# eth-ait/MultiPly

Measured on NVIDIA H100. Metric: rays/sec, higher is better.
Workload: dtype f32 (fp16 hi/lo split tensor-core operands, fp32 accumulate)

## Files before the change

### multiply_b200/csrc/mlp_tc.cu

```cuda
#include "common.cuh"
#include <vector>
#include <mutex>
#include <type_traits>
#include <stdlib.h>

namespace mp {

enum {
  K_SP_PLAIN = 0,
  K_SP_SAVE = 1,
  K_SP_SEED = 2,
  K_FEAT = 3,
  K_BWD = 4,
  K_FINAL_GRAD = 5,
  K_RELU = 6
};
enum {
  F_INJECT_EMB = 1,
  F_SDF_DOT = 2,
  F_SKIP_GRAD = 4,
  F_EXTRA_IN = 8,
  F_RGB_OUT = 16
};
constexpr int kMaxSteps = 24;
constexpr int kSlotBytes = 32768;
constexpr int kRing = 3;
constexpr int kBlobSlots = 170;

struct TcStep {
  int nk;
  int kind;
  int flags;
  int sig;
  const float* bias;
  int slot_off;
  int sc;
  int terms;
};

struct TcProgram {
  int nsteps;
  TcStep step[kMaxSteps];
  const uint4* blob;
  const float* inv_scale;
  int d_in, multires, E, inj_col, n_extra;
  const float* w8row;
  const float* b8;
  const float* Wrgb;
  const float* brgb;
};

struct TcIO : MlpCall {
  float rz;
  char* scratch;
  size_t scratch_per_cta;
};

constexpr int kConsumers = 2;
constexpr int kThreads = 128 * (1 + kConsumers);

constexpr size_t kSigBytes = (size_t)8 * kConsumers * 32 * 128 * 16;
constexpr size_t kFeatBytes = (size_t)kConsumers * 32 * 128 * 16;
constexpr size_t kGeBytes = (size_t)96 * 128 * 4;
constexpr size_t kEmbBytes = (size_t)96 * 128 * 4;
constexpr size_t kScratchPerCta = kSigBytes + kFeatBytes + kGeBytes + kEmbBytes;

constexpr int kABytes = 2 * 4 * 128 * 128;
constexpr int kSmemBytes = kABytes + kRing * kSlotBytes + 256 + 1024;
static_assert(kSmemBytes <= 232448, "shared memory budget of one CTA (227 KB)");

__device__ __forceinline__ uint32_t smem_u32(const void* p) { return (uint32_t)__cvta_generic_to_shared(p); }

__device__ __forceinline__ void mbar_init(uint64_t* bar, uint32_t count) {
  asm volatile("mbarrier.init.shared::cta.b64 [%0], %1;" ::"r"(smem_u32(bar)), "r"(count));
}
__device__ __forceinline__ void mbar_arrive(uint64_t* bar) {
  asm volatile("mbarrier.arrive.shared::cta.b64 _, [%0];" ::"r"(smem_u32(bar)) : "memory");
}
__device__ __forceinline__ void mbar_expect_tx(uint64_t* bar, uint32_t bytes) {
  asm volatile("mbarrier.arrive.expect_tx.shared::cta.b64 _, [%0], %1;" ::"r"(smem_u32(bar)), "r"(bytes) : "memory");
}
__device__ __forceinline__ void mbar_wait(uint64_t* bar, uint32_t parity) {
  asm volatile(
      "{\n"
      ".reg .pred p;\n"
      "WAIT_LOOP:\n"
      "mbarrier.try_wait.parity.shared::cta.b64 p, [%0], %1;\n"
      "@p bra WAIT_DONE;\n"
      "bra WAIT_LOOP;\n"
      "WAIT_DONE:\n"
      "}\n" ::"r"(smem_u32(bar)),
      "r"(parity)
      : "memory");
}
__device__ __forceinline__ void bulk_g2s(void* dst, const void* src, uint32_t bytes, uint64_t* bar) {
  asm volatile("cp.async.bulk.shared::cluster.global.mbarrier::complete_tx::bytes [%0], [%1], %2, [%3];" ::"r"(
                   smem_u32(dst)),
               "l"(src), "r"(bytes), "r"(smem_u32(bar))
               : "memory");
}
__device__ __forceinline__ void prefetch_l2(const void* p, uint32_t bytes) {
  asm volatile("cp.async.bulk.prefetch.L2.global [%0], %1;" ::"l"(p), "r"(bytes) : "memory");
}
__device__ __forceinline__ void fence_async_smem() { asm volatile("fence.proxy.async.shared::cta;" ::: "memory"); }

__device__ __forceinline__ void wg_sync(int id) { asm volatile("bar.sync %0, 128;" ::"r"(id) : "memory"); }

__device__ __forceinline__ void wgmma_fence() { asm volatile("wgmma.fence.sync.aligned;" ::: "memory"); }
__device__ __forceinline__ void wgmma_commit() { asm volatile("wgmma.commit_group.sync.aligned;" ::: "memory"); }
template <int N>
__device__ __forceinline__ void wgmma_wait() {
  asm volatile("wgmma.wait_group.sync.aligned %0;" ::"n"(N) : "memory");
}
__device__ __forceinline__ void acc_fence(float* d) {
#pragma unroll
  for (int i = 0; i < 128; ++i) asm volatile("" : "+f"(d[i])::"memory");
}

#define MP_D4(i) "+f"(d[i]), "+f"(d[i + 1]), "+f"(d[i + 2]), "+f"(d[i + 3])
#define MP_D16(i) MP_D4(i), MP_D4(i + 4), MP_D4(i + 8), MP_D4(i + 12)
__device__ __forceinline__ void wgmma_f16(float* d, uint64_t a_desc, uint64_t b_desc, uint32_t accumulate) {
  asm volatile(
      "{\n"
      ".reg .pred p;\n"
      "setp.ne.b32 p, %130, 0;\n"
      "wgmma.mma_async.sync.aligned.m64n256k16.f32.f16.f16 "
      "{%0, %1, %2, %3, %4, %5, %6, %7, %8, %9, %10, %11, %12, %13, %14, %15, "
      "%16, %17, %18, %19, %20, %21, %22, %23, %24, %25, %26, %27, %28, %29, %30, %31, "
      "%32, %33, %34, %35, %36, %37, %38, %39, %40, %41, %42, %43, %44, %45, %46, %47, "
      "%48, %49, %50, %51, %52, %53, %54, %55, %56, %57, %58, %59, %60, %61, %62, %63, "
      "%64, %65, %66, %67, %68, %69, %70, %71, %72, %73, %74, %75, %76, %77, %78, %79, "
      "%80, %81, %82, %83, %84, %85, %86, %87, %88, %89, %90, %91, %92, %93, %94, %95, "
      "%96, %97, %98, %99, %100, %101, %102, %103, %104, %105, %106, %107, %108, %109, %110, %111, "
      "%112, %113, %114, %115, %116, %117, %118, %119, %120, %121, %122, %123, %124, %125, %126, %127}, "
      "%128, %129, p, 1, 1, 0, 0;\n"
      "}\n"
      : MP_D16(0), MP_D16(16), MP_D16(32), MP_D16(48), MP_D16(64), MP_D16(80), MP_D16(96), MP_D16(112)
      : "l"(a_desc), "l"(b_desc), "r"(accumulate));
}
#undef MP_D16
#undef MP_D4

__device__ __forceinline__ uint64_t make_desc(uint32_t saddr) {
  return (uint64_t)((saddr >> 4) & 0x3FFF) | (1ull << 16) | ((uint64_t)(1024 >> 4) << 32) | (1ull << 62);
}

__device__ __forceinline__ uint32_t a_off(int row, int kb, int ch) {
  return (uint32_t)(kb * 16384 + row * 128 + ((ch ^ (row & 7)) << 4));
}

__device__ __forceinline__ void split2(float a, float b, uint32_t& hi, uint32_t& lo) {
  __half2 h = __floats2half2_rn(a, b);
  float2 f = __half22float2(h);
  __half2 l = __floats2half2_rn(a - f.x, b - f.y);
  hi = *(uint32_t*)&h;
  lo = *(uint32_t*)&l;
}
__device__ __forceinline__ void split8(const float* v, uint4& hi, uint4& lo) {
  split2(v[0], v[1], hi.x, lo.x);
  split2(v[2], v[3], hi.y, lo.y);
  split2(v[4], v[5], hi.z, lo.z);
  split2(v[6], v[7], hi.w, lo.w);
}

__device__ __forceinline__ void sts128(uint32_t A32, uint32_t off, const uint4& v) {
  asm volatile("st.shared.v4.b32 [%0], {%1, %2, %3, %4};" ::"r"(A32 + off), "r"(v.x), "r"(v.y), "r"(v.z), "r"(v.w));
}
__device__ __forceinline__ void store_a8(uint32_t A32, int row, int col, const float* v) {
  uint4 hi, lo;
  split8(v, hi, lo);
  uint32_t o = a_off(row, col >> 6, (col >> 3) & 7);
  sts128(A32, o, hi);
  sts128(A32, 65536 + o, lo);
}
__device__ __forceinline__ void stsm4(uint32_t addr, uint32_t a, uint32_t b, uint32_t c, uint32_t e) {
  asm volatile("stmatrix.sync.aligned.m8n8.x4.shared.b16 [%0], {%1, %2, %3, %4};" ::"r"(addr), "r"(a), "r"(b), "r"(c),
               "r"(e));
}
__device__ __forceinline__ void store_pairs(uint32_t lane_base, uint32_t lane_x, int jp, const uint4& hi, const uint4& lo) {
  const uint32_t addr = lane_base + (uint32_t)(jp >> 2) * 16384u + ((((uint32_t)(2 * jp) & 7u) ^ lane_x) << 4);
  stsm4(addr, hi.x, hi.y, hi.z, hi.w);
  stsm4(addr + 65536u, lo.x, lo.y, lo.z, lo.w);
}
__device__ __forceinline__ void store_acc16(uint32_t lane_base, uint32_t lane_x, int jp, const float* v) {
  uint4 hi, lo;
  split8(v, hi, lo);
  store_pairs(lane_base, lane_x, jp, hi, lo);
}

__device__ __forceinline__ float quad_sum(float v) {
  v += __shfl_xor_sync(0xffffffffu, v, 1);
  v += __shfl_xor_sync(0xffffffffu, v, 2);
  return v;
}

__device__ __forceinline__ float4 ld_stream(const float4* p) {
  float4 v;
  asm volatile("ld.global.cg.v4.f32 {%0,%1,%2,%3}, [%4];" : "=f"(v.x), "=f"(v.y), "=f"(v.z), "=f"(v.w) : "l"(p));
  return v;
}
__device__ __forceinline__ uint4 ld_stream(const uint4* p) {
  uint4 v;
  asm volatile("ld.global.cg.v4.u32 {%0,%1,%2,%3}, [%4];" : "=r"(v.x), "=r"(v.y), "=r"(v.z), "=r"(v.w) : "l"(p));
  return v;
}
__device__ __forceinline__ void st_stream(float4* p, const float4& v) {
  asm volatile("st.global.cg.v4.f32 [%0], {%1,%2,%3,%4};" ::"l"(p), "f"(v.x), "f"(v.y), "f"(v.z), "f"(v.w) : "memory");
}
__device__ __forceinline__ void st_stream(uint4* p, const uint4& v) {
  asm volatile("st.global.cg.v4.u32 [%0], {%1,%2,%3,%4};" ::"l"(p), "r"(v.x), "r"(v.y), "r"(v.z), "r"(v.w) : "memory");
}

__device__ __forceinline__ void discard_line(const void* p, float dep) {
  asm volatile("discard.global.L2 [%0], 128;" ::"l"(p), "f"(dep) : "memory");
}
__device__ __forceinline__ void discard_line(const void* p, uint32_t dep) {
  asm volatile("discard.global.L2 [%0], 128;" ::"l"(p), "r"(dep) : "memory");
}

__device__ __forceinline__ float ex2_approx(float x) {
  float y;
  asm("ex2.approx.ftz.f32 %0, %1;" : "=f"(y) : "f"(x));
  return y;
}
__device__ __forceinline__ float lg2_approx(float x) {
  float y;
  asm("lg2.approx.ftz.f32 %0, %1;" : "=f"(y) : "f"(x));
  return y;
}
__device__ __forceinline__ float rcp_approx(float x) {
  float y;
  asm("rcp.approx.ftz.f32 %0, %1;" : "=f"(y) : "f"(x));
  return y;
}
__device__ __forceinline__ float softplus_fast(float z) {
  float t = z * 144.26950408889634f;
  float u = ex2_approx(t);
  float y = lg2_approx(1.f + u) * 0.0069314718055994531f;
  return t > 28.853900817779268f ? z : y;
}
__device__ __forceinline__ void softplus_fast_grad(float z, float& y, float& d) {
  float t = z * 144.26950408889634f;
  float u = ex2_approx(t);
  float w = 1.f + u;
  float r = rcp_approx(w);
  float ys = lg2_approx(w) * 0.0069314718055994531f;
  bool big = t > 28.853900817779268f;
  y = big ? z : ys;
  d = big ? 1.f : u * r;
}

__device__ __forceinline__ void final_grad(const TcProgram& P, const TcIO& io, const float* acc, float isc, int q,
                                           const float* ge, const float* emb, const int (&rowt)[2],
                                           const bool (&valid)[2], const int (&pt)[2], const int (&slot)[2],
                                           float (&nrm)[2][3]) {
  const int d = P.d_in;
  float gax[2][4] = {{0.f, 0.f, 0.f, 0.f}, {0.f, 0.f, 0.f, 0.f}};
  const int nterm = 1 + 2 * P.multires;
#pragma unroll
  for (int j = 0; j < 8; ++j) {
    if (j < 2 * d) {
      const int a = j >> 1;
#pragma unroll
      for (int e = 0; e < 4; ++e) {
        const int jj = (8 * j + 2 * q + (e & 1)) & 15;
        if (jj < nterm) {
          const int h = e >> 1;
          const int fq = (jj - 1) >> 1;
          const bool is_cos = ((jj - 1) & 1) != 0;
          const int k = (jj == 0) ? a : d + 2 * fq * d + (is_cos ? d : 0) + a;
          const float pg = ge[(size_t)k * 128 + rowt[h]];
          const float tot = fmaf(acc[4 * j + e], isc, pg);
          float w = 1.f;
          if (jj > 0) {
            const float pe = emb[(size_t)(is_cos ? k - d : k + d) * 128 + rowt[h]];
            w = (float)(1 << fq) * (is_cos ? -pe : pe);
          }
          gax[h][a] = fmaf(w, tot, gax[h][a]);
        }
      }
    }
  }
#pragma unroll
  for (int h = 0; h < 2; ++h) {
#pragma unroll
    for (int a = 0; a < 4; ++a) gax[h][a] = quad_sum(gax[h][a]);
    const float gx0 = gax[h][0], gx1 = d > 1 ? gax[h][1] : 0.f, gx2 = d > 2 ? gax[h][2] : 0.f;
    if (q == 0 && io.grad && valid[h]) {
      io.grad[3 * (size_t)pt[h]] = gx0;
      io.grad[3 * (size_t)pt[h] + 1] = gx1;
      io.grad[3 * (size_t)pt[h] + 2] = gx2;
    }
    float n0 = 0.f, n1 = 0.f, n2 = 0.f;
    if (io.jinv && valid[h]) {
      const float4* J4 = (const float4*)(io.jinv + 12 * (size_t)pt[h]);
      const float4 ja = __ldg(J4), jb = __ldg(J4 + 1), jc = __ldg(J4 + 2);
      float v0 = gx0 * ja.x + gx1 * ja.w + gx2 * jb.z;
      float v1 = gx0 * ja.y + gx1 * jb.x + gx2 * jb.w;
      float v2 = gx0 * ja.z + gx1 * jb.y + gx2 * jc.x;
      float nr = fmaxf(sqrtf(v0 * v0 + v1 * v1 + v2 * v2), 1e-12f);
      const float inr = 1.f / nr;
      v0 *= inr; v1 *= inr; v2 *= inr;
      float n2r = fmaxf(sqrtf(v0 * v0 + v1 * v1 + v2 * v2), 1e-6f);
      const float in2 = 1.f / n2r;
      n0 = v0 * in2; n1 = v1 * in2; n2 = v2 * in2;
      if (q == 0 && io.nrm) {
        io.nrm[3 * (size_t)slot[h]] = n0;
        io.nrm[3 * (size_t)slot[h] + 1] = n1;
        io.nrm[3 * (size_t)slot[h] + 2] = n2;
      }
    }
    nrm[h][0] = n0;
    nrm[h][1] = n1;
    nrm[h][2] = n2;
  }
}

__global__ void __launch_bounds__(kThreads, 1) tc_chain_kernel(const __grid_constant__ TcProgram P,
                                                               const __grid_constant__ TcIO io) {
  extern __shared__ uint8_t smem_raw[];
  const int warp = threadIdx.x >> 5, lane = threadIdx.x & 31;
  char* base = (char*)(((uintptr_t)smem_raw + 1023) & ~(uintptr_t)1023);
  char* A = base;
  const uint32_t A32 = smem_u32(A);
  char* ring = base + kABytes;
  uint64_t* bars = (uint64_t*)(ring + kRing * kSlotBytes);
  uint64_t* full = bars;
  uint64_t* empty = bars + kRing;

  const int count = io.count ? min(io.cap, *io.count) : io.cap;
  const int ntiles = (count + 127) >> 7;

  if (threadIdx.x == 0) {
    for (int i = 0; i < kRing; ++i) {
      mbar_init(&full[i], 1);
      mbar_init(&empty[i], 4 * kConsumers);
    }
    asm volatile("fence.mbarrier_init.release.cluster;" ::: "memory");
  }
  __syncthreads();

  if (warp < 4) {
    asm volatile("setmaxnreg.dec.sync.aligned.u32 40;\n" ::: "memory");
    if (warp == 0 && lane == 0) {
      uint32_t it = 0;
      for (int tile = blockIdx.x; tile < ntiles; tile += gridDim.x) {
        for (int s = 0; s < P.nsteps; ++s) {
          const char* src = (const char*)P.blob + (size_t)P.step[s].slot_off * kSlotBytes;
          const int nslot = 2 * P.step[s].nk;
          const int jstep = P.step[s].terms == 1 ? 2 : 1;
          for (int j = 0; j < nslot; j += jstep, ++it) {
            int r = it % kRing;
            uint32_t ph = (it / kRing) & 1;
            mbar_wait(&empty[r], ph ^ 1);
            mbar_expect_tx(&full[r], kSlotBytes);
            bulk_g2s(ring + (size_t)r * kSlotBytes, src + (size_t)j * kSlotBytes, kSlotBytes, &full[r]);
          }
        }
      }
    }
    return;
  }
  asm volatile("setmaxnreg.inc.sync.aligned.u32 232;\n" ::: "memory");
  const int g = (warp >> 2) - 1;
  const int t = threadIdx.x & 127;
  const int wq = warp & 3, q = lane & 3;
  const int bar_id = 1 + g;
  int rowt[2];
  rowt[0] = 64 * g + 16 * wq + (lane >> 2);
  rowt[1] = rowt[0] + 8;
  const int mi = lane >> 3, rr = lane & 7;
  const uint32_t lane_base = A32 + (uint32_t)(64 * g + 16 * wq + 8 * (mi & 1) + rr) * 128u;
  const uint32_t lane_x = (uint32_t)((mi >> 1) ^ rr);
  const uint32_t a_hi = A32 + (uint32_t)g * 8192u, a_lo = a_hi + 65536u;

  char* scr = io.scratch + (size_t)blockIdx.x * io.scratch_per_cta;
  float4* sig = (float4*)scr;
  uint4* fsc = (uint4*)(scr + kSigBytes) + (size_t)g * 32 * 128;
  float* ge = (float*)(scr + kSigBytes + kFeatBytes);
  float* emb = (float*)(scr + kSigBytes + kFeatBytes + kGeBytes);
  const int d = P.d_in, E = P.E;

  float acc[128];
#pragma unroll
  for (int i = 0; i < 128; ++i) acc[i] = 0.f;
  uint32_t it = 0;

  for (int tile = blockIdx.x; tile < ntiles; tile += gridDim.x) {
    int pt[2], slot[2];
    bool valid[2];
    float x[2][4];
#pragma unroll
    for (int h = 0; h < 2; ++h) {
      pt[h] = tile * 128 + rowt[h];
      valid[h] = pt[h] < count;
      for (int a = 0; a < 4; ++a) x[h][a] = 0.f;
      if (valid[h])
        for (int a = 0; a < d; ++a) x[h][a] = io.x[(size_t)pt[h] * d + a];
      slot[h] = valid[h] ? (io.slot ? io.slot[pt[h]] : pt[h]) : 0;
    }
    {
      const int npair = d * P.multires;
      for (int pi = q; pi < npair; pi += 4) {
        const int f = pi / d, a = pi - f * d;
#pragma unroll
        for (int h = 0; h < 2; ++h) {
          float sn, cs;
          sincosf(__fmul_rn(x[h][a], (float)(1 << f)), &sn, &cs);
          emb[(size_t)(d + 2 * f * d + a) * 128 + rowt[h]] = sn;
          emb[(size_t)(d + (2 * f + 1) * d + a) * 128 + rowt[h]] = cs;
        }
      }
      if (q == 0)
        for (int a = 0; a < d; ++a)
#pragma unroll
          for (int h = 0; h < 2; ++h) emb[(size_t)a * 128 + rowt[h]] = x[h][a];
      if (io.dirs) {
        float dv[2][3];
#pragma unroll
        for (int h = 0; h < 2; ++h)
          for (int a = 0; a < 3; ++a) dv[h][a] = valid[h] ? io.dirs[(size_t)pt[h] * 3 + a] : 0.f;
        const int nvp = (P.n_extra - 3) / 2;
        for (int pi = q; pi < nvp; pi += 4) {
          const int f = pi / 3, a = pi - f * 3;
#pragma unroll
          for (int h = 0; h < 2; ++h) {
            float sn, cs;
            sincosf(__fmul_rn(dv[h][a], (float)(1 << f)), &sn, &cs);
            ge[(size_t)(3 + 6 * f + a) * 128 + rowt[h]] = sn;
            ge[(size_t)(3 + 6 * f + 3 + a) * 128 + rowt[h]] = cs;
          }
        }
        if (q == 0)
          for (int a = 0; a < 3; ++a)
#pragma unroll
            for (int h = 0; h < 2; ++h) ge[(size_t)a * 128 + rowt[h]] = dv[h][a];
      }
      __threadfence_block();
      wg_sync(bar_id);
      const int njp = P.step[0].nk * 4;
      for (int jp = 0; jp < njp; ++jp) {
        float v[8];
#pragma unroll
        for (int i = 0; i < 8; ++i) {
          const int c = 16 * jp + 8 * (i >> 2) + 2 * q + (i & 1);
          v[i] = (c < E) ? emb[(size_t)c * 128 + rowt[(i >> 1) & 1]] : 0.f;
        }
        store_acc16(lane_base, lane_x, jp, v);
      }
    }
    float nrm[2][3] = {{0.f, 0.f, 0.f}, {0.f, 0.f, 0.f}};
    for (int s = 0; s < P.nsteps; ++s) {
      const TcStep st = P.step[s];
      const float isc = P.inv_scale[st.sc] * fmaf(io.rz, (float)(4 * st.nk * (st.terms == 1 ? 1 : 3)), 1.f);
      const bool one_term = st.terms == 1;
      if (t == 0) {
        char* ws = io.scratch + (size_t)blockIdx.x * io.scratch_per_cta;
        if (st.kind == K_BWD && st.sig >= 0)
          prefetch_l2(ws + (((size_t)st.sig * kConsumers + g) * 32 * 128) * 16, 32 * 128 * 16);
        if (st.kind == K_FINAL_GRAD) prefetch_l2(ws + kSigBytes + (size_t)g * 32 * 128 * 16, 32 * 128 * 16);
      }

      fence_async_smem();
      wg_sync(bar_id);
      wgmma_fence();
      bool held = false;
      uint32_t held_slot = 0;
      auto release = [&](uint32_t slot_it) {
        if (lane == 0) mbar_arrive(&empty[slot_it % kRing]);
      };
      auto slot_issued = [&](uint32_t slot_it) {
        wgmma_commit();
        if (held) {
          wgmma_wait<1>();
          release(held_slot);
        }
        held = true;
        held_slot = slot_it;
      };
      for (int kc = 0; kc < st.nk; ++kc) {
        if (kc == 4) {
          wgmma_wait<0>();
          acc_fence(acc);
          if (held) release(held_slot);
          held = false;
#pragma unroll
          for (int h = 0; h < 2; ++h) {
#pragma unroll
            for (int c8 = 0; c8 < 16; c8 += 8) {
              const int e0 = 16 * q + c8;
              float xv[8];
#pragma unroll
              for (int j = 0; j < 8; ++j) xv[j] = 0.f;
              if (io.dirs) {
#pragma unroll
                for (int j = 0; j < 8; ++j)
                  if (e0 + j < P.n_extra) xv[j] = ge[(size_t)(e0 + j) * 128 + rowt[h]];
              } else if (e0 == 0) {
                xv[0] = x[h][0]; xv[1] = x[h][1]; xv[2] = x[h][2];
                xv[3] = nrm[h][0]; xv[4] = nrm[h][1]; xv[5] = nrm[h][2];
              }
              store_a8(A32, rowt[h], e0, xv);
            }
          }
          fence_async_smem();
          wg_sync(bar_id);
          wgmma_fence();
        }
        const uint32_t ka = (uint32_t)(kc & 3) * 16384u;
        int r = it % kRing;
        mbar_wait(&full[r], (it / kRing) & 1);
        uint32_t wb = smem_u32(ring + (size_t)r * kSlotBytes);
#pragma unroll
        for (int ks = 0; ks < 4; ++ks) {
          const uint64_t bd = make_desc(wb + ks * 32);
          wgmma_f16(acc, make_desc(a_hi + ka + ks * 32), bd, (kc | ks) != 0);
          if (!one_term) wgmma_f16(acc, make_desc(a_lo + ka + ks * 32), bd, 1);
        }
        slot_issued(it++);
        if (!one_term) {
          r = it % kRing;
          mbar_wait(&full[r], (it / kRing) & 1);
          wb = smem_u32(ring + (size_t)r * kSlotBytes);
#pragma unroll
          for (int ks = 0; ks < 4; ++ks) wgmma_f16(acc, make_desc(a_hi + ka + ks * 32), make_desc(wb + ks * 32), 1);
          slot_issued(it++);
        }
      }
      wgmma_wait<0>();
      acc_fence(acc);
      if (held) release(held_slot);

      auto reload_features = [&]() {
#pragma unroll
        for (int jp = 0; jp < 16; ++jp) {
          const uint4 fh = ld_stream(&fsc[(size_t)jp * 128 + t]);
          const uint4 fl = ld_stream(&fsc[(size_t)(16 + jp) * 128 + t]);
          store_pairs(lane_base, lane_x, jp, fh, fl);
          if ((lane & 7) == 0) {
            discard_line(&fsc[(size_t)jp * 128 + t], fh.x);
            discard_line(&fsc[(size_t)(16 + jp) * 128 + t], fl.x);
          }
        }
      };
      if (st.kind == K_FINAL_GRAD) {
        final_grad(P, io, acc, isc, q, ge, emb, rowt, valid, pt, slot, nrm);
        if (s + 1 < P.nsteps) reload_features();
        continue;
      }

      auto run_epi = [&](auto kind) {
        constexpr int KIND = decltype(kind)::value;
        float dot[2][3] = {{0.f, 0.f, 0.f}, {0.f, 0.f, 0.f}};
#pragma unroll
        for (int jp = 0; jp < 16; ++jp) {
          float* v = acc + 8 * jp;
          float yv[8];
#pragma unroll
          for (int jj = 0; jj < 2; ++jj) {
            const int j = 2 * jp + jj;
            const int c = 8 * j + 2 * q;
            float* u = v + 4 * jj;
            float b[2] = {0.f, 0.f};
            if constexpr (KIND != K_BWD) {
              const float2 b2 = __ldg((const float2*)(st.bias + c));
              b[0] = b2.x;
              b[1] = b2.y;
            }
            if constexpr (KIND == K_SP_SEED) {
              const float2 w2 = __ldg((const float2*)(P.w8row + c));
              const float w[2] = {w2.x, w2.y};
#pragma unroll
              for (int e = 0; e < 4; ++e) {
                float y, dd;
                softplus_fast_grad(fmaf(u[e], isc, b[e & 1]), y, dd);
                dot[e >> 1][0] = fmaf(y, w[e & 1], dot[e >> 1][0]);
                yv[4 * jj + e] = y;
                u[e] = dd * w[e & 1];
              }
            } else if constexpr (KIND == K_SP_SAVE || KIND == K_SP_PLAIN) {
              if constexpr (KIND == K_SP_SAVE) {
                float dd[4];
#pragma unroll
                for (int e = 0; e < 4; ++e) softplus_fast_grad(fmaf(u[e], isc, b[e & 1]), u[e], dd[e]);
                st_stream(&sig[(((size_t)st.sig * kConsumers + g) * 32 + j) * 128 + t], make_float4(dd[0], dd[1], dd[2], dd[3]));
              } else {
#pragma unroll
                for (int e = 0; e < 4; ++e) u[e] = softplus_fast(fmaf(u[e], isc, b[e & 1]));
              }
              if ((st.flags & F_INJECT_EMB) && c + 1 >= P.inj_col) {
#pragma unroll
                for (int e = 0; e < 4; ++e)
                  if (c + (e & 1) >= P.inj_col) u[e] = emb[(size_t)(c + (e & 1) - P.inj_col) * 128 + rowt[e >> 1]];
              }
              if (st.flags & F_SDF_DOT) {
                const float2 w2 = __ldg((const float2*)(P.w8row + c));
                dot[0][0] = fmaf(u[0], w2.x, fmaf(u[1], w2.y, dot[0][0]));
                dot[1][0] = fmaf(u[2], w2.x, fmaf(u[3], w2.y, dot[1][0]));
              }
            } else if constexpr (KIND == K_FEAT) {
#pragma unroll
              for (int e = 0; e < 4; ++e) u[e] = fmaf(u[e], isc, b[e & 1]);
              if (io.feat) {
#pragma unroll
                for (int h = 0; h < 2; ++h)
                  if (valid[h]) *(float2*)(io.feat + (size_t)pt[h] * 256 + c) = make_float2(u[2 * h], u[2 * h + 1]);
              }
            } else if constexpr (KIND == K_BWD) {
              float4 s4 = make_float4(1.f, 1.f, 1.f, 1.f);
              const float4* sp = &sig[(((size_t)(st.sig < 0 ? 0 : st.sig) * kConsumers + g) * 32 + j) * 128 + t];
              if (st.sig >= 0) s4 = ld_stream(sp);
              const float sv[4] = {s4.x, s4.y, s4.z, s4.w};
              if ((st.flags & F_SKIP_GRAD) && c + 1 >= P.inj_col) {
#pragma unroll
                for (int e = 0; e < 4; ++e) {
                  const float gval = u[e] * isc;
                  const int col = c + (e & 1);
                  if (col >= P.inj_col) {
                    ge[(size_t)(col - P.inj_col) * 128 + rowt[e >> 1]] = gval;
                    u[e] = 0.f;
                  } else {
                    u[e] = gval * sv[e];
                  }
                }
              } else {
#pragma unroll
                for (int e = 0; e < 4; ++e) u[e] *= isc * sv[e];
              }
              if (st.sig >= 0 && (lane & 7) == 0) discard_line(sp, s4.x);
            } else {
#pragma unroll
              for (int e = 0; e < 4; ++e) u[e] = fmaxf(fmaf(u[e], isc, b[e & 1]), 0.f);
              if (st.flags & F_RGB_OUT) {
#pragma unroll
                for (int k = 0; k < 3; ++k) {
                  const float2 w2 = __ldg((const float2*)(P.Wrgb + 256 * k + c));
                  dot[0][k] = fmaf(u[0], w2.x, fmaf(u[1], w2.y, dot[0][k]));
                  dot[1][k] = fmaf(u[2], w2.x, fmaf(u[3], w2.y, dot[1][k]));
                }
              }
            }
          }
          if constexpr (KIND == K_SP_SEED) {
            uint4 fh, fl;
            split8(yv, fh, fl);
            st_stream(&fsc[(size_t)jp * 128 + t], fh);
            st_stream(&fsc[(size_t)(16 + jp) * 128 + t], fl);
          }
          bool to_a = true;
          if constexpr (KIND == K_RELU) to_a = !(st.flags & F_RGB_OUT);
          if (to_a) store_acc16(lane_base, lane_x, jp, v);
        }
        if (st.flags & F_SDF_DOT) {
#pragma unroll
          for (int h = 0; h < 2; ++h) {
            const float sdot = quad_sum(dot[h][0]);
            if (q == 0 && valid[h] && io.sdf) io.sdf[slot[h]] = __ldg(P.b8) + sdot;
          }
        }
        if constexpr (KIND == K_RELU) {
          if (st.flags & F_RGB_OUT) {
#pragma unroll
            for (int h = 0; h < 2; ++h) {
#pragma unroll
              for (int k = 0; k < 3; ++k) {
                const float z = __ldg(P.brgb + k) + quad_sum(dot[h][k]);
                if (q == 0 && valid[h] && io.rgb) io.rgb[3 * (size_t)slot[h] + k] = 1.f / (1.f + __expf(-z));
              }
            }
          }
        }
      };
      switch (st.kind) {
        case K_SP_PLAIN: run_epi(std::integral_constant<int, K_SP_PLAIN>{}); break;
        case K_SP_SAVE: run_epi(std::integral_constant<int, K_SP_SAVE>{}); break;
        case K_SP_SEED: run_epi(std::integral_constant<int, K_SP_SEED>{}); break;
        case K_FEAT: run_epi(std::integral_constant<int, K_FEAT>{}); break;
        case K_BWD: run_epi(std::integral_constant<int, K_BWD>{}); break;
        default: run_epi(std::integral_constant<int, K_RELU>{}); break;
      }
      if (st.flags & F_SKIP_GRAD) __threadfence_block();
    }
  }
}

struct TcBlob {
  TcProgram sdf_prog;
  TcProgram full_prog;
  TcProgram fwd_prog;
  bool has_full;
};

__global__ void absmax_kernel(const float* __restrict__ W, int n, float* __restrict__ inv_scale) {
  __shared__ float s[256];
  float m = 0.f;
  for (int i = threadIdx.x; i < n; i += blockDim.x) m = fmaxf(m, fabsf(W[i]));
  s[threadIdx.x] = m;
  __syncthreads();
  for (int o = 128; o > 0; o >>= 1) {
    if (threadIdx.x < o) s[threadIdx.x] = fmaxf(s[threadIdx.x], s[threadIdx.x + o]);
    __syncthreads();
  }
  if (threadIdx.x == 0) {
    float mx = s[0];
    int ex = 0;
    if (mx > 0.f) frexpf(mx, &ex);
    float sc = ldexpf(1.f, 14 - ex);
    inv_scale[0] = 1.f / sc;
  }
}

__global__ void pack_slot_kernel(const float* __restrict__ W, int ld, int transposed, int n_off, int k_off,
                                 int n_valid, int k_valid, int kc, const float* __restrict__ inv_scale,
                                 uint8_t* __restrict__ dst_hi, uint8_t* __restrict__ dst_lo, int perm16) {
  int idx = blockIdx.x * blockDim.x + threadIdx.x;
  if (idx >= 256 * 64) return;
  int n = idx >> 6, k = idx & 63;
  int kk = kc * 64 + k;
  int ns = n;
  if (perm16) {
    const int dd = perm16, a = n >> 4, j = n & 15;
    ns = n_valid;
    if (n < 64 && a < dd) {
      const int k = (j == 0) ? a : dd + ((j - 1) >> 1) * 2 * dd + ((j - 1) & 1) * dd + a;
      if (k < n_valid) ns = k;
    }
  }
  float w = 0.f;
  if (ns < n_valid && kk < k_valid)
    w = transposed ? W[(size_t)(k_off + kk) * ld + n_off + ns] : W[(size_t)(n_off + ns) * ld + k_off + kk];
  w = __fdiv_rn(w, inv_scale[0]);
  __half h = __float2half_rn(w);
  __half l = __float2half_rn(w - __half2float(h));
  uint32_t off = (uint32_t)(n * 128 + ((((k >> 3) ^ (n & 7))) << 4) + (k & 7) * 2);
  *(__half*)(dst_hi + off) = h;
  *(__half*)(dst_lo + off) = l;
}

__global__ void copy_strided_kernel(const float* __restrict__ src, int stride, int n, float* __restrict__ dst) {
  int i = blockIdx.x * blockDim.x + threadIdx.x;
  if (i < n) dst[i] = src[(size_t)i * stride];
}

__global__ void pad_rows_kernel(const float* __restrict__ src, int lds, int nrows, int ncols, float* __restrict__ dst) {
  int i = blockIdx.x * blockDim.x + threadIdx.x;
  if (i >= nrows * 256) return;
  int r = i >> 8, c = i & 255;
  dst[i] = (c < ncols) ? src[(size_t)r * lds + c] : 0.f;
}

__global__ void fold_mm_kernel(const float* __restrict__ Wc, int ldc, int coff, const float* __restrict__ W8f, int ld8,
                               const float* __restrict__ b8f, int n_rows, float* __restrict__ M, int ldm,
                               float* __restrict__ cb) {
  int k = blockIdx.x * 16 + threadIdx.x, n = blockIdx.y * 16 + threadIdx.y;
  if (n >= n_rows || k >= 256) return;
  const float* w = Wc + (size_t)n * ldc + coff;
  double acc = 0.0;
  for (int j = 0; j < 256; ++j) acc += (double)w[j] * (double)W8f[(size_t)j * ld8 + k];
  M[(size_t)n * ldm + k] = (float)acc;
  if (k == 0) {
    double a2 = 0.0;
    for (int j = 0; j < 256; ++j) a2 += (double)w[j] * (double)b8f[j];
    cb[n] = (float)a2;
  }
}

__global__ void fill_extra_cols_kernel(const float* __restrict__ Wt, int n_out, int n_extra, float* __restrict__ M, int ldm) {
  int i = blockIdx.x * blockDim.x + threadIdx.x;
  if (i >= 256 * 64) return;
  int n = i >> 6, e = i & 63;
  M[(size_t)n * ldm + 256 + e] = (n < n_out && e < n_extra) ? Wt[(size_t)e * n_out + n] : 0.f;
}

size_t tc_pack_bytes() { return (size_t)kBlobSlots * kSlotBytes + (1 << 20); }

struct PackCtx {
  cudaStream_t st;
  uint8_t* blob;
  int nslots;
  int nlayers;
  float* inv_scale;
};

static int pack_layer(PackCtx& c, TcStep& stp, int kind, int flags, int sig, const float* bias, const float* W, int ld,
                      int transposed, int n_off, int n_valid, int k_valid, int nk, int total_elems, int perm16 = 0) {
  MP_REQUIRE(c.nslots + 2 * nk <= kBlobSlots, "tc_pack: slot budget exceeded (%d)", c.nslots + 2 * nk);
  const int layer = c.nlayers++;
  stp.nk = nk;
  stp.kind = kind;
  stp.flags = flags;
  stp.sig = sig;
  stp.bias = bias;
  stp.slot_off = c.nslots;
  stp.sc = layer;
  stp.terms = 3;
  absmax_kernel<<<1, 256, 0, c.st>>>(W, total_elems, c.inv_scale + layer);
  MP_LAUNCH_CHECK();
  for (int kc = 0; kc < nk; ++kc) {
    uint8_t* hi = c.blob + (size_t)c.nslots * kSlotBytes;
    uint8_t* lo = hi + kSlotBytes;
    pack_slot_kernel<<<64, 256, 0, c.st>>>(W, ld, transposed, n_off, 0, n_valid, k_valid, kc, c.inv_scale + layer, hi,
                                           lo, perm16);
    MP_LAUNCH_CHECK();
    c.nslots += 2;
  }
  return 0;
}

void tc_free(Field& f) {
  delete (TcBlob*)f.tc;
  f.tc = nullptr;
}

int tc_pack(Field& f, Arena& a, cudaStream_t st) {
  TcBlob* tb = new TcBlob();
  memset(tb, 0, sizeof(*tb));
  f.tc = tb;
  const int E = f.emb_dim;
  PackCtx c;
  c.st = st;
  c.nslots = 0;
  c.nlayers = 0;
  c.blob = (uint8_t*)a.take<uint4>((size_t)kBlobSlots * kSlotBytes / 16);
  c.inv_scale = a.take<float>(32);
  float* w8row = a.take<float>(256);
  float* Wrgb = a.take<float>(3 * 256);
  float* b8feat = a.take<float>(256);
  MP_REQUIRE(a.ok, "tc_pack: storage too small");
  MP_CHECK_CUDA(cudaMemsetAsync(c.blob, 0, (size_t)kBlobSlots * kSlotBytes, st));
  TcProgram P;
  memset(&P, 0, sizeof(P));
  P.blob = (const uint4*)c.blob;
  P.inv_scale = c.inv_scale;
  P.d_in = f.d_in;
  P.multires = f.multires;
  P.E = E;
  P.inj_col = kHidden - E;
  P.w8row = w8row;
  P.b8 = f.imp_b[8];
  P.Wrgb = Wrgb;
  P.n_extra = f.ren_extra;
  copy_strided_kernel<<<1, 256, 0, st>>>(f.imp_W[8], 1, 256, w8row);
  MP_LAUNCH_CHECK();
  copy_strided_kernel<<<1, 256, 0, st>>>(f.imp_b[8] + 1, 1, 256, b8feat);
  MP_LAUNCH_CHECK();
  int s = 0;
  for (int l = 0; l < 8; ++l) {
    const int in = f.imp_in[l], out = f.imp_out[l];
    const int flags = ((l == f.skip_layer - 1) ? F_INJECT_EMB : 0) | ((l == 7) ? F_SDF_DOT : 0);
    MP_TRY(pack_layer(c, P.step[s++], K_SP_PLAIN, flags, l, (l == 0) ? f.imp_b0_eff : f.imp_b[l], f.imp_W[l], in, 0,
                      0, out, (l == 0) ? E : in, (l == 0) ? (E + 63) / 64 : 4, out * in));
  }
  P.nsteps = s;
  tb->sdf_prog = P;
  tb->fwd_prog = P;
  MP_TRY(pack_layer(c, tb->fwd_prog.step[s], K_FEAT, 0, -1, b8feat, f.imp_W[8], 256, 0, 1, 256, 256, 4, 257 * 256));
  tb->fwd_prog.nsteps = s + 1;
  const bool fg_chain = (f.ren_mode == 0) && (f.n_ren == 5) && f.ren_out[0] == 256;
  const bool bg_chain = (f.ren_mode == 1) && (f.n_ren == 2) && f.ren_out[0] <= 256 && f.ren_extra <= 27;
  tb->has_full = fg_chain || bg_chain;
  constexpr int kLdM = 320;
  float* Mfold = a.take<float>(256 * kLdM);
  f.ren_cb = a.take<float>(264);
  f.ren_b0_fold = a.take<float>(264);
  MP_REQUIRE(a.ok, "tc_pack: storage too small");
  if (tb->has_full) {
    const int in0 = f.ren_in[0] == 0 ? 0 : (f.ren_mode == 0 ? 6 + 8 + 256 : f.ren_extra + 32 + 256);
    const int coff = f.ren_mode == 0 ? 14 : f.ren_extra + 32;
    const int o0 = f.ren_out[0];
    fold_mm_kernel<<<dim3(256 / 16, div_up(o0, 16)), dim3(16, 16), 0, st>>>(f.ren_W[0], in0, coff, f.imp_W[8] + 256, 256,
                                                                          f.imp_b[8] + 1, o0, Mfold, kLdM, f.ren_cb);
    MP_LAUNCH_CHECK();
    MP_REQUIRE(f.ren_extra <= 64, "tc_pack: more than 64 extra colour inputs");
    fill_extra_cols_kernel<<<64, 256, 0, st>>>(f.ren_Wt[0], o0, f.ren_extra, Mfold, kLdM);
    MP_LAUNCH_CHECK();
  }
  if (bg_chain) {
    const int o0 = f.ren_out[0];
    MP_TRY(pack_layer(c, P.step[s++], K_RELU, F_EXTRA_IN | F_RGB_OUT, -1, f.ren_b0_fold, Mfold, kLdM, 0, 0, o0, kLdM, 5,
                      256 * kLdM));
    pad_rows_kernel<<<div_up(3 * 256, 256), 256, 0, st>>>(f.ren_W[1], o0, 3, o0, Wrgb);
    MP_LAUNCH_CHECK();
    P.brgb = f.ren_b[1];
    P.nsteps = s;
    tb->full_prog = P;
  }
  if (fg_chain) {
    for (int l = 0; l < 8; ++l) P.step[l].kind = (l == 7) ? K_SP_SEED : K_SP_SAVE;
    for (int l = 7; l >= 1; --l) {
      const int in = f.imp_in[l], out = f.imp_out[l];
      MP_TRY(pack_layer(c, P.step[s++], K_BWD, (l == f.skip_layer) ? F_SKIP_GRAD : 0, l - 1, nullptr, f.imp_W[l], in, 1,
                        0, in, out, 4, out * in));
    }
    MP_REQUIRE(f.d_in <= 4 && 1 + 2 * f.multires <= 14,
               "tc_pack: the final-gradient step keeps 1 + 2 * multires <= 14 embedding columns per axis");
    MP_TRY(pack_layer(c, P.step[s++], K_FINAL_GRAD, 0, -1, nullptr, f.imp_W[0], f.imp_in[0], 1, 0, E, 256, 4,
                      256 * f.imp_in[0], f.d_in));
    MP_TRY(pack_layer(c, P.step[s++], K_RELU, F_EXTRA_IN, -1, f.ren_b0_fold, Mfold, kLdM, 0, 0, 256, kLdM, 5,
                      256 * kLdM));
    for (int l = 1; l < 4; ++l)
      MP_TRY(pack_layer(c, P.step[s++], K_RELU, (l == 3) ? F_RGB_OUT : 0, -1, f.ren_b[l], f.ren_W[l], 256, 0, 0, 256,
                        256, 4, 256 * 256));
    MP_CHECK_CUDA(cudaMemcpyAsync(Wrgb, f.ren_W[4], (size_t)3 * 256 * sizeof(float), cudaMemcpyDeviceToDevice, st));
    P.brgb = f.ren_b[4];
    P.nsteps = s;
    tb->full_prog = P;
  }
  return 0;
}

size_t tc_workspace_bytes(int N) { return (size_t)sm_count() * kScratchPerCta + 4096; }

struct ProfEntry {
  cudaEvent_t e0, e1;
  int kind;
  int cap;
  int* host_count;
};
static std::mutex g_prof_mu;
static std::atomic<bool> g_prof_on{false};
static std::vector<ProfEntry>* g_prof = nullptr;
static int* g_prof_pinned = nullptr;
static int g_prof_used = 0;
constexpr int kProfMax = 1 << 16;

int prof_enable(int on) {
  std::lock_guard<std::mutex> g(g_prof_mu);
  if (on && !g_prof) {
    g_prof = new std::vector<ProfEntry>();
    MP_CHECK_CUDA(cudaMallocHost(&g_prof_pinned, kProfMax * sizeof(int)));
  }
  g_prof_on = on != 0;
  return 0;
}
int prof_read(double* ms, long long* launches, double* points, int reset) {
  for (int k = 0; k < 4; ++k) {
    ms[k] = 0;
    launches[k] = 0;
    points[k] = 0;
  }
  std::lock_guard<std::mutex> g(g_prof_mu);
  if (!g_prof) return 0;
  for (auto& e : *g_prof) {
    MP_CHECK_CUDA(cudaEventSynchronize(e.e1));
    float t = 0.f;
    MP_CHECK_CUDA(cudaEventElapsedTime(&t, e.e0, e.e1));
    ms[e.kind] += t;
    launches[e.kind] += 1;
    int n = e.host_count ? *e.host_count : e.cap;
    points[e.kind] += (double)(n < e.cap ? n : e.cap);
  }
  if (reset) {
    for (auto& e : *g_prof) {
      cudaEventDestroy(e.e0);
      cudaEventDestroy(e.e1);
    }
    g_prof->clear();
    g_prof_used = 0;
  }
  return 0;
}

std::atomic<int> g_precision{0};

constexpr float kRzPerMma = 1.72e-8f;

static int tc_launch(const TcProgram& P0, TcIO io, void* ws, size_t ws_bytes, cudaStream_t st, MlpProg kind) {
  TcProgram P = P0;
  {
    const int mode = g_precision.load();
    for (int s = 0; s < P.nsteps; ++s)
      P.step[s].terms = (mode == 2 || (mode == 1 && P.step[s].kind == K_RELU)) ? 1 : 3;
  }
  int grid = sm_count();
  {
    static int grid_override = -1;
    if (grid_override < 0) {
      const char* eg = getenv("MP_TC_GRID");
      grid_override = eg ? atoi(eg) : 0;
    }
    if (grid_override > 0 && grid_override < grid) grid = grid_override;
  }
  int maxtiles = (io.cap + 127) / 128;
  if (grid > maxtiles) grid = maxtiles;
  if (grid < 1) return 0;
  MP_REQUIRE(ws && ws_bytes >= (size_t)grid * kScratchPerCta, "tensor-core engine: workspace too small (%zu < %zu)",
             ws_bytes, (size_t)grid * kScratchPerCta);
  io.scratch = (char*)ws;
  io.scratch_per_cta = kScratchPerCta;
  static const float rz_scale = [] {
    const char* er = getenv("MP_TC_RZ_SCALE");
    return er ? (float)atof(er) : 1.f;
  }();
  io.rz = kRzPerMma * rz_scale;
  {
    static std::mutex attr_mu;
    static unsigned long long attr_done = 0;
    int dev = 0;
    MP_CHECK_CUDA(cudaGetDevice(&dev));
    std::lock_guard<std::mutex> g(attr_mu);
    if (dev < 0 || dev >= 64 || !((attr_done >> dev) & 1ull)) {
      MP_CHECK_CUDA(cudaFuncSetAttribute(tc_chain_kernel, cudaFuncAttributeMaxDynamicSharedMemorySize, kSmemBytes));
      if (dev >= 0 && dev < 64) attr_done |= 1ull << dev;
    }
  }
  ProfEntry pe;
  std::unique_lock<std::mutex> prof_lock(g_prof_mu, std::defer_lock);
  if (g_prof_on.load()) prof_lock.lock();
  const bool prof = prof_lock.owns_lock() && g_prof_on.load() && g_prof && g_prof_used < kProfMax;
  if (prof) {
    MP_CHECK_CUDA(cudaEventCreate(&pe.e0));
    MP_CHECK_CUDA(cudaEventCreate(&pe.e1));
    pe.kind = (int)kind;
    pe.cap = io.cap;
    pe.host_count = nullptr;
    if (io.count) {
      pe.host_count = g_prof_pinned + g_prof_used++;
      MP_CHECK_CUDA(cudaMemcpyAsync(pe.host_count, io.count, sizeof(int), cudaMemcpyDeviceToHost, st));
    }
    MP_CHECK_CUDA(cudaEventRecord(pe.e0, st));
  }
  tc_chain_kernel<<<grid, kThreads, kSmemBytes, st>>>(P, io);
  MP_LAUNCH_CHECK();
  if (prof) {
    MP_CHECK_CUDA(cudaEventRecord(pe.e1, st));
    g_prof->push_back(pe);
  }
  return 0;
}

int tc_run(const Field& f, const MlpCall& c, void* ws, size_t ws_bytes, cudaStream_t st) {
  MP_REQUIRE(f.tc, "tensor-core engine: field not packed");
  const TcBlob& tb = *(const TcBlob*)f.tc;
  const MlpProg prog = mlp_prog(c);
  TcIO io{};
  static_cast<MlpCall&>(io) = c;
  if (prog == MlpProg::kSdf) return tc_launch(tb.sdf_prog, io, ws, ws_bytes, st, prog);
  if (prog == MlpProg::kForward) return tc_launch(tb.fwd_prog, io, ws, ws_bytes, st, prog);
  if (prog == MlpProg::kBg) {
    MP_REQUIRE(tb.has_full && f.ren_mode == 1, "tensor-core engine: not a background field");
    return tc_launch(tb.full_prog, io, ws, ws_bytes, st, prog);
  }
  MP_REQUIRE(tb.has_full, "tensor-core engine: this field has no fused shading program");
  if (c.feat) {
    TcIO fio{};
    fio.x = c.x;
    fio.slot = c.slot;
    fio.count = c.count;
    fio.cap = c.cap;
    fio.feat = c.feat;
    MP_TRY(tc_launch(tb.fwd_prog, fio, ws, ws_bytes, st, MlpProg::kForward));
    io.feat = nullptr;
  }
  return tc_launch(tb.full_prog, io, ws, ws_bytes, st, prog);
}

}
```

Measured before the change: 447,000.

## Use narrower wgmma N and partial weight transfers for layers with few output columns

Adds m64n128 and m64n64 wgmma variants and records each layer's live output-column count at pack time. Narrow layers then issue smaller MMAs and have the producer bulk-copy only ncols*128 bytes per weight slot instead of the full 32KB. The 256-wide path is also specialised at compile time on one-term versus three-term. Unused accumulator registers are zeroed afterwards, which adds code size and register pressure from the templated lambda instantiations.

Measured after the change: 452,500 (median of 6 runs). 1.01x the previous value.

```diff
diff --git a/multiply_b200/csrc/mlp_tc.cu b/multiply_b200/csrc/mlp_tc.cu
--- a/multiply_b200/csrc/mlp_tc.cu
+++ b/multiply_b200/csrc/mlp_tc.cu
@@ -36,6 +36,7 @@
   int slot_off;
   int sc;
   int terms;
+  int ncols;
 };
 
 struct TcProgram {
@@ -138,8 +139,43 @@
       : MP_D16(0), MP_D16(16), MP_D16(32), MP_D16(48), MP_D16(64), MP_D16(80), MP_D16(96), MP_D16(112)
       : "l"(a_desc), "l"(b_desc), "r"(accumulate));
 }
+__device__ __forceinline__ void wgmma_f16_n128(float* d, uint64_t a_desc, uint64_t b_desc, uint32_t accumulate) {
+  asm volatile(
+      "{\n"
+      ".reg .pred p;\n"
+      "setp.ne.b32 p, %66, 0;\n"
+      "wgmma.mma_async.sync.aligned.m64n128k16.f32.f16.f16 "
+      "{%0, %1, %2, %3, %4, %5, %6, %7, %8, %9, %10, %11, %12, %13, %14, %15, "
+      "%16, %17, %18, %19, %20, %21, %22, %23, %24, %25, %26, %27, %28, %29, %30, %31, "
+      "%32, %33, %34, %35, %36, %37, %38, %39, %40, %41, %42, %43, %44, %45, %46, %47, "
+      "%48, %49, %50, %51, %52, %53, %54, %55, %56, %57, %58, %59, %60, %61, %62, %63}, "
+      "%64, %65, p, 1, 1, 0, 0;\n"
+      "}\n"
+      : MP_D16(0), MP_D16(16), MP_D16(32), MP_D16(48)
+      : "l"(a_desc), "l"(b_desc), "r"(accumulate));
+}
+__device__ __forceinline__ void wgmma_f16_n64(float* d, uint64_t a_desc, uint64_t b_desc, uint32_t accumulate) {
+  asm volatile(
+      "{\n"
+      ".reg .pred p;\n"
+      "setp.ne.b32 p, %34, 0;\n"
+      "wgmma.mma_async.sync.aligned.m64n64k16.f32.f16.f16 "
+      "{%0, %1, %2, %3, %4, %5, %6, %7, %8, %9, %10, %11, %12, %13, %14, %15, "
+      "%16, %17, %18, %19, %20, %21, %22, %23, %24, %25, %26, %27, %28, %29, %30, %31}, "
+      "%32, %33, p, 1, 1, 0, 0;\n"
+      "}\n"
+      : MP_D16(0), MP_D16(16)
+      : "l"(a_desc), "l"(b_desc), "r"(accumulate));
+}
 #undef MP_D16
 #undef MP_D4
+template <int N>
+__device__ __forceinline__ void wgmma_cols(float* d, uint64_t a_desc, uint64_t b_desc, uint32_t accumulate) {
+  static_assert(N == 64 || N == 128 || N == 256, "wgmma N");
+  if constexpr (N == 256) wgmma_f16(d, a_desc, b_desc, accumulate);
+  else if constexpr (N == 128) wgmma_f16_n128(d, a_desc, b_desc, accumulate);
+  else wgmma_f16_n64(d, a_desc, b_desc, accumulate);
+}
 
 __device__ __forceinline__ uint64_t make_desc(uint32_t saddr) {
   return (uint64_t)((saddr >> 4) & 0x3FFF) | (1ull << 16) | ((uint64_t)(1024 >> 4) << 32) | (1ull << 62);
@@ -349,12 +385,13 @@
           const char* src = (const char*)P.blob + (size_t)P.step[s].slot_off * kSlotBytes;
           const int nslot = 2 * P.step[s].nk;
           const int jstep = P.step[s].terms == 1 ? 2 : 1;
+          const uint32_t bytes = (uint32_t)P.step[s].ncols * 128;
           for (int j = 0; j < nslot; j += jstep, ++it) {
             int r = it % kRing;
             uint32_t ph = (it / kRing) & 1;
             mbar_wait(&empty[r], ph ^ 1);
-            mbar_expect_tx(&full[r], kSlotBytes);
-            bulk_g2s(ring + (size_t)r * kSlotBytes, src + (size_t)j * kSlotBytes, kSlotBytes, &full[r]);
+            mbar_expect_tx(&full[r], bytes);
+            bulk_g2s(ring + (size_t)r * kSlotBytes, src + (size_t)j * kSlotBytes, bytes, &full[r]);
           }
         }
       }
@@ -478,58 +515,84 @@
         held = true;
         held_slot = slot_it;
       };
-      for (int kc = 0; kc < st.nk; ++kc) {
-        if (kc == 4) {
-          wgmma_wait<0>();
-          acc_fence(acc);
-          if (held) release(held_slot);
-          held = false;
-#pragma unroll
-          for (int h = 0; h < 2; ++h) {
-#pragma unroll
-            for (int c8 = 0; c8 < 16; c8 += 8) {
-              const int e0 = 16 * q + c8;
-              float xv[8];
-#pragma unroll
-              for (int j = 0; j < 8; ++j) xv[j] = 0.f;
-              if (io.dirs) {
-#pragma unroll
-                for (int j = 0; j < 8; ++j)
-                  if (e0 + j < P.n_extra) xv[j] = ge[(size_t)(e0 + j) * 128 + rowt[h]];
-              } else if (e0 == 0) {
-                xv[0] = x[h][0]; xv[1] = x[h][1]; xv[2] = x[h][2];
-                xv[3] = nrm[h][0]; xv[4] = nrm[h][1]; xv[5] = nrm[h][2];
+      auto mma_chunks = [&](auto n_c, auto terms_c) {
+        constexpr int N = decltype(n_c)::value;
+        constexpr int TERMS = decltype(terms_c)::value;
+        const bool three = TERMS == 3 || (TERMS == 0 && !one_term);
+        for (int kc = 0; kc < st.nk; ++kc) {
+          if (N != 64 && kc == 4) {
+            wgmma_wait<0>();
+            acc_fence(acc);
+            if (held) release(held_slot);
+            held = false;
+#pragma unroll
+            for (int h = 0; h < 2; ++h) {
+#pragma unroll
+              for (int c8 = 0; c8 < 16; c8 += 8) {
+                const int e0 = 16 * q + c8;
+                float xv[8];
+#pragma unroll
+                for (int j = 0; j < 8; ++j) xv[j] = 0.f;
+                if (io.dirs) {
+#pragma unroll
+                  for (int j = 0; j < 8; ++j)
+                    if (e0 + j < P.n_extra) xv[j] = ge[(size_t)(e0 + j) * 128 + rowt[h]];
+                } else if (e0 == 0) {
+                  xv[0] = x[h][0]; xv[1] = x[h][1]; xv[2] = x[h][2];
+                  xv[3] = nrm[h][0]; xv[4] = nrm[h][1]; xv[5] = nrm[h][2];
+                }
+                store_a8(A32, rowt[h], e0, xv);
               }
-              store_a8(A32, rowt[h], e0, xv);
+            }
+            fence_async_smem();
+            wg_sync(bar_id);
+            wgmma_fence();
+          }
+          const uint32_t ka = (uint32_t)(kc & 3) * 16384u;
+          int r = it % kRing;
+          mbar_wait(&full[r], (it / kRing) & 1);
+          uint32_t wb = smem_u32(ring + (size_t)r * kSlotBytes);
+          if (!three) {
+#pragma unroll
+            for (int ks = 0; ks < 4; ++ks)
+              wgmma_cols<N>(acc, make_desc(a_hi + ka + ks * 32), make_desc(wb + ks * 32), (kc | ks) != 0);
+          } else {
+#pragma unroll
+            for (int ks = 0; ks < 4; ++ks) {
+              const uint64_t bd = make_desc(wb + ks * 32);
+              wgmma_cols<N>(acc, make_desc(a_hi + ka + ks * 32), bd, (kc | ks) != 0);
+              wgmma_cols<N>(acc, make_desc(a_lo + ka + ks * 32), bd, 1);
             }
           }
-          fence_async_smem();
-          wg_sync(bar_id);
-          wgmma_fence();
+          slot_issued(it++);
+          if (three) {
+            r = it % kRing;
+            mbar_wait(&full[r], (it / kRing) & 1);
+            wb = smem_u32(ring + (size_t)r * kSlotBytes);
+#pragma unroll
+            for (int ks = 0; ks < 4; ++ks)
+              wgmma_cols<N>(acc, make_desc(a_hi + ka + ks * 32), make_desc(wb + ks * 32), 1);
+            slot_issued(it++);
+          }
         }
-        const uint32_t ka = (uint32_t)(kc & 3) * 16384u;
-        int r = it % kRing;
-        mbar_wait(&full[r], (it / kRing) & 1);
-        uint32_t wb = smem_u32(ring + (size_t)r * kSlotBytes);
-#pragma unroll
-        for (int ks = 0; ks < 4; ++ks) {
-          const uint64_t bd = make_desc(wb + ks * 32);
-          wgmma_f16(acc, make_desc(a_hi + ka + ks * 32), bd, (kc | ks) != 0);
-          if (!one_term) wgmma_f16(acc, make_desc(a_lo + ka + ks * 32), bd, 1);
-        }
-        slot_issued(it++);
-        if (!one_term) {
-          r = it % kRing;
-          mbar_wait(&full[r], (it / kRing) & 1);
-          wb = smem_u32(ring + (size_t)r * kSlotBytes);
-#pragma unroll
-          for (int ks = 0; ks < 4; ++ks) wgmma_f16(acc, make_desc(a_hi + ka + ks * 32), make_desc(wb + ks * 32), 1);
-          slot_issued(it++);
-        }
-      }
+      };
+      using runtime_terms = std::integral_constant<int, 0>;
+      if (st.ncols == 64)
+        mma_chunks(std::integral_constant<int, 64>{}, runtime_terms{});
+      else if (st.ncols == 128)
+        mma_chunks(std::integral_constant<int, 128>{}, runtime_terms{});
+      else if (one_term)
+        mma_chunks(std::integral_constant<int, 256>{}, std::integral_constant<int, 1>{});
+      else
+        mma_chunks(std::integral_constant<int, 256>{}, std::integral_constant<int, 3>{});
       wgmma_wait<0>();
       acc_fence(acc);
       if (held) release(held_slot);
+      if (st.ncols < 256) {
+#pragma unroll
+        for (int i = 32; i < 128; ++i)
+          if (2 * i >= st.ncols) acc[i] = 0.f;
+      }
 
       auto reload_features = [&]() {
 #pragma unroll
@@ -794,6 +857,9 @@
   stp.slot_off = c.nslots;
   stp.sc = layer;
   stp.terms = 3;
+  const int live = perm16 ? 16 * perm16 : n_valid;
+  stp.ncols = live <= 64 ? 64 : live <= 128 ? 128 : 256;
+  MP_REQUIRE(stp.ncols > 64 || nk <= 4, "tc_pack: a 64-column step has no extra-input K-block");
   absmax_kernel<<<1, 256, 0, c.st>>>(W, total_elems, c.inv_scale + layer);
   MP_LAUNCH_CHECK();
   for (int kc = 0; kc < nk; ++kc) {
```
